# bigpon/QPNet

Measured on AMD Instinct MI355X. Metric: train steps/sec (batch-1 chunk-steps of RF+20000 samples, aggregate over GPUs), higher is better.
Workload: dtype f32; 1 GPU; config[1]: paper-size SI-QPNet (C=64,S=256,4F+4A) training step, forward+CE+backward+Adam on one chunk of 20900 samples (RF 946 + batch_length 19954), batch 1 per GPU; global_batch=1, parallelism=dp1 (utterance-sharded chunks, one flat-gradient all-reduce per step), backend=none, world_size=1, aux_1x1=frame rate (hoisted: K = 128 + one 4-deep step)

## Files before the change

qpnet_amd/csrc/train_bwd.hip:

```cpp
#include "train_common.h"
#include "train_post.h"
#include "qpn_handle.h"
#include <string.h>
#include <stdlib.h>
#include <math.h>

template <int MT>
__global__ __launch_bounds__(512) void k_post_bwd(TrainParams p, TrainBwd bw) {
    constexpr int TM = 16 * MT;
    extern __shared__ float sm[];
    const int S = p.S, Q = p.Q, LC = p.LC;
    const int ldp = tr_lda(Q > S ? Q : S), ldr = tr_lda(S);
    float* P = sm; float* R = sm + TM * ldp;
    const int b = blockIdx.y, t0 = blockIdx.x * TM;
    const int tid = threadIdx.x, lane = tid & 63, wave = tid >> 6;
    const int NTS = S / 16;
    const int npairs = (NTS + 1) / 2;
    const int np0 = wave < npairs ? wave : 0;
    const int pnt[2] = {2 * np0, (2 * np0 + 1 < NTS) ? 2 * np0 + 1 : 2 * np0};
    float my[2][MT][4], ms[2][MT][4];
    auto mask_load = [&](const float* src, float (&m)[2][MT][4]) {
#pragma unroll
        for (int j = 0; j < 2; ++j)
#pragma unroll
// ... 964 lines not shown
            a += ((v[0] + v[1]) + (v[2] + v[3])) + ((v[4] + v[5]) + (v[6] + v[7]));
        }
        for (; c < nch; ++c) a += sp[(size_t)c * gstage];
        a *= scale;
        for (int k = k0; k < k1; ++k) g[gdst_list[k]] = a;
        return;
    }
    if (!tail) return;
    const int64_t j = i - s1;
    if (j < n_gzero) g[gzero[j]] = 0.f;
    else if (append_scale && j < n_gzero + 4 && !(flag_again && j == n_gzero + 1)) g[n + (j - n_gzero)] = j == n_gzero ? scale : (j == n_gzero + 1 && status && *status) ? 1.f : 0.f;
}

__global__ __launch_bounds__(256) void k_causal_bwd(TrainParams p, TrainBwd bw, int rows_per_wg, int CB) {
    extern __shared__ float tab[];
    const int C = p.C, Q = p.Q;
    const int tid = threadIdx.x;
    const int64_t total = (int64_t)p.B * p.N1;
    const int64_t r0 = (int64_t)blockIdx.x * rows_per_wg, r1 = r0 + rows_per_wg < total ? r0 + rows_per_wg : total;
    for (int cb = 0; cb < C; cb += CB) {
        const int cbv = C - cb < CB ? C - cb : CB;
        for (int i = tid; i < 2 * Q * CB; i += 256) tab[i] = 0.f;
        __syncthreads();
        const int cpr = cbv;
        for (int64_t idx = r0 * cpr + tid; idx < r1 * cpr; idx += 256) {
            const int64_t rr = idx / cpr; const int c = (int)(idx - rr * cpr);
            const int b = (int)(rr / p.N1), n = (int)(rr - (int64_t)b * p.N1);
            const size_t o = ((size_t)b * p.N1 + n) * C + cb + c;
            const float v = bw.DXA[0][o] + bw.DXB[0][o];
            const int64_t xo = (int64_t)p.T - p.N0 + n;
            int64_t s0 = p.x[(size_t)b * p.T + xo] % Q, s1 = p.x[(size_t)b * p.T + xo + 1] % Q;
            if (s0 < 0) s0 += Q;
            if (s1 < 0) s1 += Q;
            atomicAdd(&tab[(0 * Q + s0) * CB + c], v);
            atomicAdd(&tab[(1 * Q + s1) * CB + c], v);
        }
        __syncthreads();
        for (int i = tid; i < 2 * Q * cbv; i += 256) {
            const int c = i / (2 * Q), qt = i - c * 2 * Q, q = qt >> 1, tp = qt & 1;
            const float v = tab[(tp * Q + q) * CB + c];
            if (v != 0.f) atomicAdd(&bw.gflat[p.causal_w + ((size_t)(cb + c) * Q + q) * 2 + tp], v * bw.gscale);
        }
        for (int c = tid; c < cbv; c += 256) {
            float s = 0.f;
            for (int q = 0; q < Q; ++q) s += tab[(0 * Q + q) * CB + c];
            atomicAdd(&bw.gflat[p.causal_b + cb + c], s * bw.gscale);
        }
        __syncthreads();
    }
}

__global__ __launch_bounds__(128) void k_up_bwd(UpArgs u) { up_bwd_body(u, blockIdx.x, blockIdx.y, threadIdx.x, 128); }

__global__ __launch_bounds__(128) void k_aux_tail(AuxArgs p) {
    __shared__ float hrow[1024];
    __shared__ float red[2];
    const AuxGeom& ag = p.g;
    const int C = p.C, A = p.A, L = p.L, tid = threadIdx.x;
    const int bx = blockIdx.x;
    float v = 0.f;
    const bool role_a = bx < L * A;
    if (role_a) {
        const int l = bx / A, a = bx - l * A, n = tid;
        const size_t wi = (n < C ? ag.auxS[l] + (size_t)n * A : ag.auxT[l] + (size_t)(n - C) * A) + a;
        const float va = p.flat[wi];
        float e = 0.f;
        {
            float ev[TR_EB_SLOTS];
#pragma unroll
            for (int k = 0; k < TR_EB_SLOTS; ++k) ev[k] = p.EB[(size_t)(l * TR_EB_SLOTS + k) * 2 * C + n];
#pragma unroll
            for (int k = 0; k < TR_EB_SLOTS; ++k) e += ev[k];
        }
        float acc = 0.f;
        for (int b = 0; b < p.B; ++b) {
            const float* hb = p.h + ((size_t)b * A + a) * p.F + p.ffirst;
            const float* D = p.DPA + (size_t)(l * p.B + b) * (p.nfr + 1) * 2 * C + n;
            for (int f0 = 0; f0 < p.nfr; f0 += 1024) {
                const int nf = p.nfr - f0 < 1024 ? p.nfr - f0 : 1024;
                __syncthreads();
                for (int i = tid; i < nf; i += 128) hrow[i] = hb[f0 + i];
                __syncthreads();
                int f = 0;
                for (; f + 64 <= nf; f += 64) {
                    float d[64];
#pragma unroll
                    for (int k = 0; k < 64; ++k) d[k] = D[(size_t)(f0 + f + k) * 2 * C];
#pragma unroll
                    for (int k = 0; k < 64; ++k) acc += d[k] * hrow[f + k];
                }
                for (; f + 16 <= nf; f += 16) {
                    float d[16];
#pragma unroll
                    for (int k = 0; k < 16; ++k) d[k] = D[(size_t)(f0 + f + k) * 2 * C];
#pragma unroll
                    for (int k = 0; k < 16; ++k) acc += d[k] * hrow[f + k];
                }
                for (; f < nf; ++f) acc += D[(size_t)(f0 + f) * 2 * C] * hrow[f];
            }
        }
        p.gflat[wi] = (acc + p.flat[p.up_b] * e) * p.gscale;
        v = va * e;
    } else {
        const int j = bx - L * A;
        const int q0 = p.F * p.U - p.N1;
        const int items = L * p.B * p.nfr;
        for (int it = tid; it < items; it += 128) {
            const int fx = it % p.nfr, lb = it / p.nfr, l = lb / p.B;
            const int n = (p.ffirst + fx) * p.U + j - q0;
            if (n >= ag.s_out[l] && n < p.N1) v += p.GW[(size_t)lb * p.N1 + n];
        }
    }
    for (int sft = 32; sft >= 1; sft >>= 1) v += __shfl_xor(v, sft);
    if ((tid & 63) == 0) red[tid >> 6] = v;
    __syncthreads();
    if (tid == 0) {
        if (role_a) atomicAdd(p.gflat + p.up_b, (red[0] + red[1]) * p.gscale);
        else p.gflat[p.up_w + (bx - L * A)] = (red[0] + red[1]) * p.gscale;
    }
}

__device__ __forceinline__ void zero_dx_slice(const TrainParams& p, const TrainBwd& bw, int j, int b, size_t part, size_t nparts, int t, int nthr) {
    const int C = p.C;
    const TrLayer ly = p.layers[j];
    const size_t nDX = (size_t)p.B * p.N1 * C;
    float* A = bw.DXA[0] + (size_t)j * nDX + (size_t)b * p.N1 * C;
    float* Bq = bw.DXB[0] + (size_t)j * nDX + (size_t)b * p.N1 * C;
    const int a0 = j == 0 ? 0 : ly.s_in, a1 = ly.s_out;
    const int b0 = ly.adaptive ? 0 : p.N1 - ly.dilation, b1 = p.N1;
    const size_t na = (size_t)(a1 - a0) * C / 4, nb = (size_t)(b1 > b0 ? b1 - b0 : 0) * C / 4;
    const float4 z = make_float4(0.f, 0.f, 0.f, 0.f);
    const size_t nh = p.hoist ? (size_t)(p.nfr + 1) * 2 * C / 4 : (j == 0 ? (size_t)p.N1 * p.Ap / 4 : 0);
    const size_t ne = (p.hoist && b == 0) ? (size_t)TR_EB_SLOTS * 2 * C / 4 : 0;
    float* H = p.hoist ? bw.DPA + (size_t)(j * p.B + b) * (p.nfr + 1) * 2 * C : bw.DHUP + (size_t)b * p.N1 * p.Ap;
    for (size_t i = part * nthr + t; i < na + nb + nh + ne; i += nparts * nthr) {
        if (i < na) ((float4*)(A + (size_t)a0 * C))[i] = z;
        else if (i < na + nb) ((float4*)(Bq + (size_t)(b0 > 0 ? b0 : 0) * C))[i - na] = z;
        else if (i < na + nb + nh) ((float4*)H)[i - na - nb] = z;
        else ((float4*)(bw.EB + (size_t)j * TR_EB_SLOTS * 2 * C))[i - na - nb - nh] = z;
    }
}
__global__ void k_zero_dx(TrainParams p, TrainBwd bw) {
    zero_dx_slice(p, bw, blockIdx.y, blockIdx.z, blockIdx.x, gridDim.x, threadIdx.x, blockDim.x);
}

void qpn_launch_zero_dx(const TrainParams& p, const TrainBwd& bw, hipStream_t stream) {
    hipLaunchKernelGGL(k_zero_dx, dim3(64, p.L, p.B), dim3(256), 0, stream, p, bw);
}

static void launch_reduce_early(const TrainBwd& bw, hipStream_t st, int tail, int nch_side) {
    const TrainSlabs& sl = *bw.sl;
    const int64_t n = (int64_t)(sl.g_early1 - sl.g_early0) + (tail ? bw.n_gzero + 4 : 0);
    hipLaunchKernelGGL(k_reduce_grad_s, dim3((unsigned)((n + 255) / 256)), dim3(256), 0, st, bw.slab, bw.gdst, bw.gdst_list, bw.gzero, bw.n_gzero,
                       nch_side, bw.gstage, bw.n_params, bw.gflat, bw.gscale, bw.append_scale, sl.g_early0, sl.g_early1, 0, 0, tail, bw.status, 0);
}
static void launch_up_bwd(const TrainParams& p, const TrainBwd& bw, hipStream_t st) {
    const UpArgs u = up_args(p, bw);
    hipLaunchKernelGGL(k_up_bwd, dim3(u.nfr, p.B), dim3(128), 0, st, u);
}

static void launch_aux_tail(const TrainParams& p, const TrainBwd& bw, const AuxGeom& ag, hipStream_t st) {
    hipLaunchKernelGGL(k_aux_tail, dim3(p.L * p.A + p.U), dim3(128), 0, st, tr_aux_args(p, &bw, ag));
}

int qpn_launch_grad_tail(const TrainParams& p, const TrainBwd& bw, const AuxGeom* ag, hipStream_t stream, bool early_done, bool up_done) {
    const int C = p.C, Q = p.Q, B = p.B, N1 = p.N1;
    const TrainSlabs& sl = *bw.sl;
    hipLaunchKernelGGL(k_reduce_grad_s, dim3((unsigned)(((int64_t)bw.gstage + (up_done ? 0 : bw.n_gzero + 4) + 255) / 256)), dim3(256), 0, stream, bw.slab, bw.gdst, bw.gdst_list, bw.gzero, bw.n_gzero,
                       bw.nch, bw.gstage, bw.n_params, bw.gflat, bw.gscale, bw.append_scale, 0, bw.gstage, early_done ? sl.g_early0 : 0, early_done ? sl.g_early1 : 0, up_done ? 0 : 1, bw.status, bw.append_scale == 1 ? 1 : 0);
    {
        const int64_t total = (int64_t)B * N1;
        const int nwg = 128, rpw = (int)((total + nwg - 1) / nwg);
        if (sl.g_cw < 0) {
            int CB = C < 64 ? C : 64;
            while (CB > 1 && (size_t)2 * Q * CB * sizeof(float) > 128 * 1024) CB /= 2;
            const size_t lds_c = (size_t)2 * Q * CB * sizeof(float);
            if (lds_c > 160 * 1024) { qpn_set_error("causal-table gradient: n_quantize too large for the LDS histogram"); return QPN_EINVAL; }
            if (lds_c > 48 * 1024) QPN_HIP(hipFuncSetAttribute((const void*)k_causal_bwd, hipFuncAttributeMaxDynamicSharedMemorySize, (int)lds_c));
            hipLaunchKernelGGL(k_causal_bwd, dim3(nwg), dim3(256), lds_c, stream, p, bw, rpw, CB);
        }
        if (p.U > 0 && !up_done && !p.hoist) launch_up_bwd(p, bw, stream);
        if (p.hoist && ag && !up_done) launch_aux_tail(p, bw, *ag, stream);
        if (bw.dh && !up_done) qpn_launch_input_grad(p, bw, ag, stream);
    }
    qpn_prof_mark(PG_GRAD_TAIL, stream);
    QPN_HIP(hipGetLastError());
    return QPN_OK;
}

bool qpn_stack_bwd_fits(const TrainParams& p);
int qpn_launch_stack_bwd(const TrainParams& p, const TrainBwd& bw, const StackQ& q, const TrainKnobs& k, hipStream_t stream);

void qpn_launch_post_fb(const TrainParams& p, const TrainBwd& bw, hipStream_t stream) {
    constexpr int MTW = 5;
    const size_t ldsw = (size_t)16 * MTW * (tr_lda(256) + 2 * tr_lda(64)) * sizeof(float);
    (void)hipFuncSetAttribute((const void*)k_post_fb_w<MTW>, hipFuncAttributeMaxDynamicSharedMemorySize, (int)ldsw);
    hipLaunchKernelGGL((k_post_fb_w<MTW>), dim3((p.BL + 16 * MTW - 1) / (16 * MTW), p.B), dim3(512), ldsw, stream, p, bw, 1);
}

int qpn_launch_bwd(const TrainParams& p, const TrainBwd& bw, const TrainKnobs& k, const AuxGeom& ag, const StackQ* sq, hipStream_t stream, bool post_done) {
    const int C = p.C, S = p.S, Q = p.Q, L = p.L, B = p.B, N1 = p.N1, BL = p.BL;
    const TrainSlabs& sl = *bw.sl;
    const bool off32 = N1 < (1 << 24) && (int64_t)N1 * (p.LC > 2 * C ? p.LC : 2 * C) < (1ll << 32);
    const bool persist = C == 64 && (p.Ktp == 176 || p.hoist) && p.Ap <= 64 && off32 && k.persist_bwd;
    const bool stack_q = persist && k.stack_q_bwd && sq && sq->flags && p.qctl && qpn_stack_bwd_fits(p);
    const bool wr_summed = stack_q;
    const size_t nDX = (size_t)B * N1 * C;
    const size_t lds_post = (size_t)16 * (tr_lda(Q > S ? Q : S) + tr_lda(S)) * sizeof(float);
    const size_t lds_layer = (size_t)16 * (4 * tr_lda(C) + tr_lda(2 * C)) * sizeof(float);
    if (lds_post > 160 * 1024 || lds_layer > 160 * 1024) { qpn_set_error("backward tiles do not fit LDS"); return QPN_EINVAL; }
    hipStream_t side = bw.side; hipEvent_t ev_fork = bw.ev_fork, ev_join = bw.ev_join;
    const bool overlap = side && !qpn_prof_serial() && !k.serial;
    const bool post_wide = S == 256 && Q == 256 && C == 64 && (p.LC == 256 || p.LC == 512) && k.post_wide;
    const bool zero_in_post = post_wide && k.zero_in_post;
    if (post_done) { }
    else if (!zero_in_post) qpn_launch_zero_dx(p, bw, stream);
    if (post_done) { }
    else if (post_wide) {
        constexpr int MTW = 5;
        const size_t ldsw = (size_t)16 * MTW * tr_lda(256) * sizeof(float);
        QPN_HIP(hipFuncSetAttribute((const void*)k_post_bwd_w<MTW>, hipFuncAttributeMaxDynamicSharedMemorySize, (int)ldsw));
        hipLaunchKernelGGL((k_post_bwd_w<MTW>), dim3((BL + 16 * MTW - 1) / (16 * MTW), B), dim3(512), ldsw, stream, p, bw, zero_in_post ? 1 : 0);
    } else {
        if (lds_post > 48 * 1024) (void)hipFuncSetAttribute((const void*)k_post_bwd<1>, hipFuncAttributeMaxDynamicSharedMemorySize, (int)lds_post);
        hipLaunchKernelGGL((k_post_bwd<1>), dim3((BL + 15) / 16, B), dim3(512), lds_post, stream, p, bw);
    }
    qpn_prof_mark(PG_POST_BWD, stream);
    const int nch = bw.nch;
    int nch_side_ = nch;
    const bool gen = k.wgrad_generic;
    Wg2 wbase; memset(&wbase, 0, sizeof(wbase));
    wbase.slab = bw.slab; wbase.gstage = bw.gstage; wbase.nb = B; wbase.C = C; wbase.Ap = p.Ap; wbase.hup = p.HUP; wbase.tap = p.TAP; wbase.ncol_groups = 1;
    bool ok = true;
    auto launch_skip_post = [&](hipStream_t st) {
        Wg2 w = wbase;
// ... 55 lines not shown
    }
    if (overlap) {
        QPN_HIP(hipEventRecord(ev_fork, stream));
        QPN_HIP(hipStreamWaitEvent(side, ev_fork, 0));
        qpn_prof_mark(-1, side);
        launch_skip_post(side);
        if (early_reduce) { launch_reduce_early(bw, side, up_side ? 1 : 0, nch_side_); qpn_prof_mark(PG_GRAD_TAIL, side); }
        if (early_reduce && up_side && bw.ev_early && bw.early_recorded) { QPN_HIP(hipEventRecord(bw.ev_early, side)); *bw.early_recorded = 1; }
    }
    const int swz = k.xcd_swizzle ? 1 : 0;
    if (p.hoist && !persist) { qpn_set_error("internal: the frame-rate aux term needs the register-resident layer kernels"); return QPN_EINVAL; }
    if (stack_q) {
        const int rcq = qpn_launch_stack_bwd(p, bw, *sq, k, stream);
        if (rcq) return rcq;
    }
    for (int l = L - 1; l >= 0 && !stack_q; --l) {
        const TrLayer& ly = p.layers[l];
        const int rows = N1 - ly.s_out;
        const int tiles = (rows + 15) / 16;
        if (persist) {
            int G = qpn_num_cus() * 2; if (G > tiles) G = tiles;
            if (G > 1024) G = 1024;
            const size_t ldsp = (size_t)(8 * 16 * tr_lda(C) + 16 * tr_lda(2 * C) + 16 * tr_lda(p.Ktp) + 64) * sizeof(float);
            const bool last = l == L - 1;
            const void* kf = p.hoist ? (last ? (const void*)k_layer_bwd_p<8, true> : (const void*)k_layer_bwd_p<8, false>)
                                     : (last ? (const void*)k_layer_bwd_p<11, true> : (const void*)k_layer_bwd_p<11, false>);
            (void)hipFuncSetAttribute(kf, hipFuncAttributeMaxDynamicSharedMemorySize, (int)ldsp);
            if (p.hoist) {
                if (last) hipLaunchKernelGGL((k_layer_bwd_p<8, true>), dim3(G, B), dim3(256), ldsp, stream, p, bw, l, swz ? 2 : 0, tiles, p.scratch_rows);
                else hipLaunchKernelGGL((k_layer_bwd_p<8, false>), dim3(G, B), dim3(256), ldsp, stream, p, bw, l, swz ? 2 : 0, tiles, p.scratch_rows);
            } else {
                if (last) hipLaunchKernelGGL((k_layer_bwd_p<11, true>), dim3(G, B), dim3(256), ldsp, stream, p, bw, l, swz ? 2 : 0, tiles, p.scratch_rows);
                else hipLaunchKernelGGL((k_layer_bwd_p<11, false>), dim3(G, B), dim3(256), ldsp, stream, p, bw, l, swz ? 2 : 0, tiles, p.scratch_rows);
            }
        } else {
            if (lds_layer > 48 * 1024) (void)hipFuncSetAttribute((const void*)k_layer_bwd<1>, hipFuncAttributeMaxDynamicSharedMemorySize, (int)lds_layer);
            hipLaunchKernelGGL((k_layer_bwd<1>), dim3(tiles, B), dim3(256), lds_layer, stream, p, bw, l, l == L - 1 ? 1 : 0, swz);
        }
    }
    auto build_causal = [&]() {
        Wg2 w = wbase;
        w.nlayers = 2; w.ncol_groups = Q / (Q % 64 == 0 ? 64 : 128);      w.bmode = 4; w.xc = p.XC; w.B1 = w.B2 = nullptr; w.B_lstride = 0;
        w.A = bw.DXA[0]; w.A2 = bw.DXB[0]; w.A_lstride = 0; w.lda = C; w.M = C; w.rowsA = N1;
        w.N = Q; w.Nvalid = Q; w.rowsB = N1 + 1; w.ldb = 0; w.ldc = Q;
        for (int tp = 0; tp < 2; ++tp) { w.row0A[tp] = 0; w.row0B[tp] = tp; w.R[tp] = N1; w.goff[tp] = sl.g_cw + tp * C * Q; w.gbias[tp] = tp == 0 ? sl.g_cb : -1; w.tap_off[tp] = -1; w.dil[tp] = 0; }
        return w;
    };
    const bool wr_side = overlap && k.wr_side;
    if (wr_side || up_side) {
        QPN_HIP(hipEventRecord(bw.ev_mid, stream));
        QPN_HIP(hipStreamWaitEvent(side, bw.ev_mid, 0));
        qpn_prof_mark(-1, side);
        if (up_side) {
            if (p.hoist) launch_aux_tail(p, bw, ag, side); else launch_up_bwd(p, bw, side);
            if (bw.dh) qpn_launch_input_grad(p, bw, &ag, side);
            qpn_prof_mark(PG_GRAD_TAIL, side);
        }
        if (wr_side) { ok = ok && wgrad2_any(build_wr(), nch, gen, side); qpn_prof_mark(PG_WGRAD_WR, side); }
    }
    if (overlap) QPN_HIP(hipEventRecord(ev_join, side));
    qpn_prof_mark(PG_LAYER_BWD, stream);
    ok = ok && wgrad2_any(build_w1(), nch, gen, stream);
    qpn_prof_mark(PG_WGRAD, stream);
    if (!wr_side) { ok = ok && wgrad2_any(build_wr(), nch, gen, stream); qpn_prof_mark(PG_WGRAD_WR, stream); }
    if (!overlap) launch_skip_post(stream);
    if (sl.g_cw >= 0) ok = ok && wgrad2_any(build_causal(), nch, gen, stream);
    qpn_prof_mark(PG_WGRAD_CAUSAL, stream);
    if (overlap) { QPN_HIP(hipStreamWaitEvent(stream, ev_join, 0)); qpn_prof_mark(-1, stream); }
    if (!ok) { qpn_set_error("weight-gradient tiles: unsupported geometry (n_resch <= 128 on this path; wider stacks take the GEMM path)"); return QPN_EINVAL; }
    return qpn_launch_grad_tail(p, bw, &ag, stream, early_reduce, up_side);
}
```

qpnet_amd/csrc/train_gemm.hip:

```cpp
#include "train_common.h"
#include "qpn_handle.h"
#include <string.h>

typedef float f32x16 __attribute__((ext_vector_type(16)));

#define GM 128
#define GN 128
#ifndef GK
#define GK 16
#endif
#ifndef GKT
#define GKT 16
#endif
#define G_LDA (GK + 1)
#ifndef GEMM_WAVES
#define GEMM_WAVES
#endif
#define G_LDB 128

enum { AL_PLAIN = 0, AL_SUM2 = 1, AL_RELU = 2 };
enum { EP_BIAS = 0, EP_GATE, EP_RES, EP_MASK, EP_DZ, EP_DA, EP_STORE };

struct GArgs {
    int M, N, K, nb;
// ... 401 lines not shown
    { AuxGeom ag0; memset(&ag0, 0, sizeof(ag0)); qpn_launch_prep(p, ag0, stream); }
    qpn_prof_mark(PG_PREP, stream);
    for (int l = 0; l < L; ++l) {
        const TrLayer& ly = p.layers[l];
        const int rows = N1 - ly.s_out;
        {
            GArgs g = gbase(p);
            g.M = rows; g.N = 2 * C; g.K = w.K1; g.row_base = ly.s_out;
            const float* Xin = p.X + (size_t)l * nDX;
            g.a[0] = Xin; g.a_ld[0] = C; g.a_kend[0] = C; g.a_kvalid[0] = C; g.a_tap[0] = 0; g.a_row0[0] = ly.s_out; g.a_bs[0] = (long)N1 * C;
            g.a[1] = Xin; g.a_ld[1] = C; g.a_kend[1] = 2 * C; g.a_kvalid[1] = C; g.a_tap[1] = 1; g.a_row0[1] = 0; g.a_bs[1] = (long)N1 * C;
            g.a[2] = p.HUP; g.a_ld[2] = p.Ap; g.a_kend[2] = w.K1; g.a_kvalid[2] = p.Ap; g.a_tap[2] = 0; g.a_row0[2] = ly.s_out; g.a_bs[2] = (long)N1 * p.Ap;
            g.tap = ly.adaptive ? p.TAP + ly.tap_off : nullptr; g.tap_bs = N1; g.dil = ly.dilation;
            g.b = w.wp + w.w1[l]; g.ldb = w.N1g;
            g.bias = p.bp + ly.bias1;
            g.o[0] = p.SG + (size_t)l * nDX; g.o[1] = p.TH + (size_t)l * nDX; g.o[2] = w.G + (size_t)l * nDX; g.o_bs = (long)N1 * C; g.o_ld = C; g.o_row0 = ly.s_out;
            launch_nn<AL_PLAIN, EP_GATE>(g, w.N1g / GN, stream);
        }
        if (l + 1 < L) {
            GArgs g = gbase(p);
            g.M = rows; g.N = C; g.K = C; g.row_base = ly.s_out;
            g.a[0] = w.G + (size_t)l * nDX; g.a_ld[0] = C; g.a_kvalid[0] = C; g.a_row0[0] = ly.s_out; g.a_bs[0] = (long)N1 * C;
            g.b = w.wp + w.wr[l]; g.ldb = w.Cg;
            g.bias = p.bp + ly.biasr;
            g.o[0] = p.X + (size_t)(l + 1) * nDX; g.o_bs = (long)N1 * C; g.o_ld = C; g.o_row0 = ly.s_out;
            g.e[0] = p.X + (size_t)l * nDX; g.e_bs = (long)N1 * C; g.e_ld = C; g.e_row0 = ly.s_out;
            launch_nn<AL_PLAIN, EP_RES>(g, w.Cg / GN, stream);
        }
    }
    qpn_prof_mark(PG_LAYER_FWD, stream);
    {
        GArgs g = gbase(p);
        g.M = BL; g.N = S; g.K = L * C; g.row_base = N1 - BL;
        g.a[0] = w.G; g.a_ld[0] = C; g.a_kvalid[0] = L * C; g.a_row0[0] = N1 - BL; g.a_bs[0] = (long)N1 * C;
        g.a_rep_len = C; g.a_rep_stride = (long)nDX;
        g.b = w.wp + w.ws; g.ldb = w.Sg; g.bias = p.bp + p.bias_s;
        g.o[0] = p.S0; g.o_bs = (long)BL * S; g.o_ld = S; g.o_row0 = 0;
        launch_nn<AL_PLAIN, EP_BIAS>(g, w.Sg / GN, stream);
        g = gbase(p);
        g.M = BL; g.N = S; g.K = S; g.a[0] = p.S0; g.a_ld[0] = S; g.a_kvalid[0] = S; g.a_bs[0] = (long)BL * S;
        g.b = w.wp + w.p1; g.ldb = w.Sg; g.bias = p.bp + p.bias_p1;
        g.o[0] = p.Y0; g.o_bs = (long)BL * S; g.o_ld = S;
        launch_nn<AL_RELU, EP_BIAS>(g, w.Sg / GN, stream);
        g.N = Q; g.a[0] = p.Y0; g.b = w.wp + w.p2; g.ldb = w.Qg; g.bias = p.bp + p.bias_p2;
        g.o[0] = p.logits; g.o_bs = (long)BL * Q; g.o_ld = Q;
        launch_nn<AL_RELU, EP_BIAS>(g, w.Qg / GN, stream);
    }
    qpn_prof_mark(PG_POST_FWD, stream);
    QPN_HIP(hipGetLastError());
    return QPN_OK;
}

void qpn_launch_zero_dx(const TrainParams& p, const TrainBwd& bw, hipStream_t stream);
int qpn_launch_grad_tail(const TrainParams& p, const TrainBwd& bw, const AuxGeom* ag, hipStream_t stream, bool early_done, bool up_done);

static void launch_post_wgrad_gemm(const TrainParams& p, const TrainBwd& bw, hipStream_t stream) {
    TArgs a; memset(&a, 0, sizeof(a));
    a.nb = p.B; a.nsplit = bw.nch; a.slab = bw.slab; a.gstage = bw.gstage; a.C = p.C; a.Ap = p.Ap;
    a.M = p.Q; a.N = p.S; a.a = bw.dlogits; a.lda = p.Q; a.rowsA = p.BL; a.b1 = p.Y0; a.ldb = p.S; a.rowsB = p.BL; a.ldc = p.S;
    a.R[0] = p.BL; a.goff[0] = bw.sl->g_p2; a.gbias[0] = bw.sl->g_bp2; a.tap_off[0] = -1;
    launch_tn<BM_RELU>(a, 1, stream);
    a.M = p.S; a.a = bw.DY0; a.lda = p.S; a.b1 = p.S0; a.goff[0] = bw.sl->g_p1; a.gbias[0] = bw.sl->g_bp1;
    launch_tn<BM_RELU>(a, 1, stream);
}

int qpn_launch_bwd_gemm(const TrainParams& p, const TrainBwd& bw, const TrainGemm& w, hipStream_t stream) {
    const int C = p.C, S = p.S, Q = p.Q, L = p.L, B = p.B, N1 = p.N1, BL = p.BL;
    const size_t nDX = (size_t)B * N1 * C;
    qpn_launch_zero_dx(p, bw, stream);
    {
        GArgs g = gbase(p);
        g.M = BL; g.N = S; g.K = Q; g.a[0] = bw.dlogits; g.a_ld[0] = Q; g.a_kvalid[0] = Q; g.a_bs[0] = (long)BL * Q;
        g.b = w.wp + w.p2t; g.ldb = w.Sg;
        g.o[0] = bw.DY0; g.o_bs = (long)BL * S; g.o_ld = S; g.e[0] = p.Y0; g.e_bs = (long)BL * S; g.e_ld = S;
        launch_nn<AL_PLAIN, EP_MASK>(g, w.Sg / GN, stream);
        g.K = S; g.a[0] = bw.DY0; g.a_ld[0] = S; g.a_kvalid[0] = S; g.a_bs[0] = (long)BL * S;
        g.b = w.wp + w.p1t; g.o[0] = bw.DS0; g.e[0] = p.S0;
        launch_nn<AL_PLAIN, EP_MASK>(g, w.Sg / GN, stream);
        g = gbase(p);
        g.M = BL; g.N = L * C; g.K = S; g.a[0] = bw.DS0; g.a_ld[0] = S; g.a_kvalid[0] = S; g.a_bs[0] = (long)BL * S;
        g.b = w.wp + w.wst; g.ldb = w.LCg;
        g.o[0] = bw.DGS; g.o_bs = (long)BL * L * C; g.o_ld = L * C;
        launch_nn<AL_PLAIN, EP_STORE>(g, w.LCg / GN, stream);
    }
    qpn_prof_mark(PG_POST_BWD, stream);
    for (int l = L - 1; l >= 0; --l) {
        const TrLayer& ly = p.layers[l];
        const int rows = N1 - ly.s_out;
        const bool last = l == L - 1;
        float* DZl = bw.DZ + (size_t)l * B * N1 * 2 * C;
        {
            GArgs g = gbase(p);
            g.M = rows; g.N = C; g.K = last ? 0 : C; g.row_base = ly.s_out;
            g.a[0] = bw.DXA[0] + (size_t)(l + 1) * nDX; g.a2 = bw.DXB[0] + (size_t)(l + 1) * nDX;
            g.a_ld[0] = C; g.a_kvalid[0] = C; g.a_row0[0] = ly.s_out; g.a_bs[0] = (long)N1 * C;
            g.b = w.wp + w.wrt[l]; g.ldb = w.Cg;
            g.o[0] = DZl; g.o_bs = (long)N1 * 2 * C; g.o_ld = 2 * C; g.o_row0 = ly.s_out;
            g.e[0] = p.SG + (size_t)l * nDX; g.e[1] = p.TH + (size_t)l * nDX; g.e_bs = (long)N1 * C; g.e_ld = C; g.e_row0 = ly.s_out;
            g.e3 = bw.DGS; g.e3_bs = (long)BL * L * C; g.e3_ld = L * C; g.e3_col0 = l * C; g.e3_rowmin = N1 - BL;
            launch_nn<AL_SUM2, EP_DZ>(g, w.Cg / GN, stream);
        }
        {
            GArgs g = gbase(p);
            g.M = rows; g.N = 2 * C + p.Ap; g.K = 2 * C; g.row_base = ly.s_out;
            g.a[0] = DZl; g.a_ld[0] = 2 * C; g.a_kvalid[0] = 2 * C; g.a_row0[0] = ly.s_out; g.a_bs[0] = (long)N1 * 2 * C;
            g.b = w.wp + w.w1t[l]; g.ldb = w.Ktg;
            g.tap = ly.adaptive ? p.TAP + ly.tap_off : nullptr; g.tap_bs = N1; g.dil = ly.dilation; g.adaptive = ly.adaptive; g.last = last;
            g.o[0] = bw.DXA[0] + (size_t)l * nDX; g.o_bs = (long)N1 * C; g.o_ld = C;
            g.e[0] = bw.DXA[0] + (size_t)(l + 1) * nDX; g.e[1] = bw.DXB[0] + (size_t)(l + 1) * nDX; g.e_bs = (long)N1 * C; g.e_ld = C; g.e_row0 = ly.s_out;
            g.db = bw.DXB[0] + (size_t)l * nDX; g.db_bs = (long)N1 * C;
            g.dh = bw.DHUP; g.dh_bs = (long)N1 * p.Ap;
            launch_nn<AL_PLAIN, EP_DA>(g, w.Ktg / GN, stream);
        }
    }
    qpn_prof_mark(PG_LAYER_BWD, stream);
    TArgs t; memset(&t, 0, sizeof(t));
    t.nb = B; t.nsplit = bw.nch; t.slab = bw.slab; t.gstage = bw.gstage; t.hup = p.HUP; t.tap = p.TAP; t.C = C; t.Ap = p.Ap;
    {
        TArgs a = t;
        a.M = 2 * C; a.N = 2 * C + p.Ap; a.a = bw.DZ; a.a_ls = (long)B * N1 * 2 * C; a.lda = 2 * C; a.rowsA = N1;
        a.b1 = p.X; a.b_ls = (long)nDX; a.ldb = C; a.rowsB = N1; a.ldc = p.Ktp;
        for (int l = 0; l < L; ++l) {
            const TrLayer& ly = p.layers[l];
            a.row0A[l] = a.row0B[l] = ly.s_out; a.R[l] = N1 - ly.s_out; a.goff[l] = bw.sl->g_w1[l]; a.gbias[l] = bw.sl->g_b1[l];
            a.tap_off[l] = ly.adaptive ? ly.tap_off : -1; a.dil[l] = ly.dilation;
        }
        launch_tn<BM_GATHER>(a, L, stream);
    }
    {
        TArgs a = t;
        a.M = C; a.N = C; a.a = bw.DXA[0] + nDX; a.a2 = bw.DXB[0] + nDX; a.a_ls = (long)nDX; a.lda = C; a.rowsA = N1;
        a.b1 = w.G; a.b_ls = (long)nDX; a.ldb = C; a.rowsB = N1; a.ldc = C;
        for (int l = 0; l < L; ++l) {
            a.row0A[l] = a.row0B[l] = p.layers[l].s_out; a.R[l] = l == L - 1 ? 0 : N1 - p.layers[l].s_out;
            a.goff[l] = bw.sl->g_wr[l]; a.gbias[l] = bw.sl->g_br[l]; a.tap_off[l] = -1;
        }
        launch_tn<BM_PLAIN>(a, L, stream);
    }
    {
        TArgs a = t;
        a.M = S; a.N = C; a.a = bw.DS0; a.a_ls = 0; a.lda = S; a.rowsA = BL;
        a.b1 = w.G; a.b_ls = (long)nDX; a.ldb = C; a.rowsB = N1; a.ldc = C;
        for (int l = 0; l < L; ++l) { a.row0A[l] = 0; a.row0B[l] = N1 - BL; a.R[l] = BL; a.goff[l] = bw.sl->g_ws[l]; a.gbias[l] = l == 0 ? bw.sl->g_bs : -1; a.tap_off[l] = -1; }
        launch_tn<BM_PLAIN>(a, L, stream);
    }
    launch_post_wgrad_gemm(p, bw, stream);
    qpn_prof_mark(PG_WGRAD, stream);
    return qpn_launch_grad_tail(p, bw, nullptr, stream, false, false);
}
```

qpnet_amd/csrc/train_host.hip:

```cpp
#include "train_common.h"
#include "qpn_handle.h"
#include <algorithm>
#include <memory>
#include <string.h>

int qpn_launch_fwd(const TrainParams& p, const TrainKnobs& k, const AuxGeom& ag, const StackQ* sq, hipStream_t stream, const TrainBwd* fuse_post_bwd, const RefreshArgs* rf);
bool qpn_step_prep_fits(const TrainParams& p);
void qpn_stack_fill(TrainParams& p);
static CeOpts ce_opts_of(const qpn_loss_opts& o, double* mass, double* d_mass);
int qpn_launch_bwd(const TrainParams& p, const TrainBwd& bw, const TrainKnobs& k, const AuxGeom& ag, const StackQ* sq, hipStream_t stream, bool post_done);
int qpn_launch_fwd_gemm(const TrainParams& p, const TrainGemm& w, hipStream_t stream);
int qpn_launch_bwd_gemm(const TrainParams& p, const TrainBwd& bw, const TrainGemm& w, hipStream_t stream);

#define LOSS_SLOT 72
static double loss_sum(const double* parts) { double sum = 0.0; for (int i = 0; i < 64; ++i) sum += parts[i]; return sum; }

struct TrainState {
    TrainLayout lay;
    int64_t n_map = 0;
    int* d_wmap = nullptr; float* d_wp = nullptr; int* d_bstart = nullptr; int* d_blist = nullptr; float* d_bp = nullptr;
    int* d_gdst = nullptr; int* d_gdst_list = nullptr; int* d_gzero = nullptr; int n_gzero = 0;
    TrainParams tp = {};
    TrainBwd bw = {};
    TrainKnobs knobs = {};
// ... 3 lines not shown
    double* d_loss3 = nullptr;
    double* d_mass = nullptr;
    int* d_status = nullptr; double* d_loss = nullptr;
    hipStream_t last_stream = nullptr;
    int* h_status_pinned = nullptr; hipEvent_t ev_status[2] = {}; bool status_pending[2] = {}; int status_newest = 0;
    double* h_loss_pinned = nullptr; hipEvent_t ev_loss[2] = {}; bool loss_pending[2] = {}; int loss_newest = 0;
    double* d_gnorm = nullptr; bool gnorm_last = false;
    bool gnorm_slot[2] = {};
    double gnorm_collected = 0.0; bool gnorm_collected_valid = false;
    bool fwd_valid = false;
    bool loss_clear = false;
    int* d_ctmap = nullptr; float* d_ct = nullptr;
    int* d_gmap = nullptr; float* d_gwp = nullptr;
    TrainGemm gm = {};
    int64_t generation = 0;
    hipStream_t side = nullptr; hipEvent_t ev_fork = nullptr, ev_join = nullptr, ev_mid = nullptr;
    hipEvent_t ev_early = nullptr; int early_recorded = 0;
    int64_t bwd_generation = -1;
    const float* post_bwd_dlogits = nullptr;
    bool post_bwd_done = false;
    bool stack_disabled = false;
    unsigned* d_sq = nullptr; size_t sq_pos_cap = 0, sq_per_dir = 0;
    StackQ sqf = {}, sqb = {};
};

static int env_int(const char* name, int dflt) { const char* e = getenv(name); return (e && *e) ? atoi(e) : dflt; }
void qpn_train_knobs_parse(TrainKnobs& k) {
    k.serial = env_int("QPN_TRAIN_SERIAL", 0) != 0;
    k.stack_q_fwd = env_int("QPN_STACK_QUEUE", 1) != 0;
    k.stack_q_bwd = k.stack_q_fwd && env_int("QPN_STACK_QUEUE_BWD", 1) != 0;
    k.stack_wgs = env_int("QPN_STACK_WGS", 0); if (k.stack_wgs < 0 || k.stack_wgs > 4096) k.stack_wgs = 0;
    k.stack_wgs_bwd = env_int("QPN_STACK_WGS_BWD", 0); if (k.stack_wgs_bwd < 0 || k.stack_wgs_bwd > 4096) k.stack_wgs_bwd = 0;
    k.persist_fwd = env_int("QPN_LAYER_PERSIST", 1) != 0;
    k.persist_bwd = env_int("QPN_LAYER_BWD_PERSIST", 1) != 0;
    k.wgrad_generic = getenv("QPN_WGRAD_GENERIC") != nullptr;
    k.wgrad_chunks = env_int("QPN_WGRAD_CHUNKS", 0); if (k.wgrad_chunks < 1 || k.wgrad_chunks > 512) k.wgrad_chunks = 0;
    k.wgrad_chunks_side = env_int("QPN_WGRAD_CHUNKS_SIDE", 0); if (k.wgrad_chunks_side < 1 || k.wgrad_chunks_side > 512) k.wgrad_chunks_side = 0;
    k.up_side = env_int("QPN_UP_SIDE", 1) != 0;
    k.reduce_early = env_int("QPN_REDUCE_EARLY", 1) != 0;
    k.wr_side = env_int("QPN_WR_SIDE", 1) != 0;
    k.post_fuse = env_int("QPN_POST_FUSE", 1) != 0;
    k.post_pair = env_int("QPN_POST_WGRAD_PAIR", 1) != 0;
    k.zero_in_post = env_int("QPN_ZERO_IN_POST", 1) != 0;
    k.post_wide = env_int("QPN_POST_WIDE", 1) != 0;
    k.xcd_swizzle = getenv("QPN_NO_XCD_SWIZZLE") == nullptr;
    k.ce_separate = getenv("QPN_CE_SEPARATE") != nullptr;
    k.event_fence = env_int("QPN_EVENT_FENCE", 0) == 1;
    k.aux_hoist = env_int("QPN_AUX_HOIST", 1) != 0;
    k.prep_fuse = env_int("QPN_PREP_FUSE", 1) != 0;
    k.test_stack_gives_up = false;
#ifdef QPN_TESTING
    k.test_stack_gives_up = env_int("QPN_TEST_STACK_GIVES_UP", 0) == 1;
#endif
}

int qpn_num_cus() {
    static int cached[64] = {0};
    int dev = 0;
    if (hipGetDevice(&dev) != hipSuccess || dev < 0 || dev >= 64) return 256;
    if (!cached[dev]) { int n = 0; if (hipDeviceGetAttribute(&n, hipDeviceAttributeMultiprocessorCount, dev) != hipSuccess || n < 1) n = 256; cached[dev] = n; }
    return cached[dev];
}

struct Prof { bool on = false; bool overlapped = false; std::vector<hipEvent_t> ev; std::vector<int> grp; std::vector<hipStream_t> st; size_t used = 0; };
static thread_local Prof g_prof;
bool qpn_prof_active() { return g_prof.on; }
bool qpn_prof_serial() { return g_prof.on && !g_prof.overlapped; }
void qpn_prof_mark(int group, hipStream_t stream) {
    Prof& P = g_prof;
    if (!P.on) return;
    if (P.used == P.ev.size()) { hipEvent_t e; if (hipEventCreate(&e) != hipSuccess) return; P.ev.push_back(e); P.grp.push_back(0); P.st.push_back(nullptr); }
    P.grp[P.used] = group; P.st[P.used] = stream;
    (void)hipEventRecord(P.ev[P.used++], stream);
}
extern "C" int qpn_train_profile_begin(qpn_handle* h, void* stream) {
    (void)h; g_prof.on = true; g_prof.overlapped = false; g_prof.used = 0;
    qpn_prof_mark(-1, (hipStream_t)stream);
    return QPN_OK;
}
extern "C" int qpn_train_profile_begin_overlapped(qpn_handle* h, void* stream) {
    (void)h; g_prof.on = true; g_prof.overlapped = true; g_prof.used = 0;
    qpn_prof_mark(-1, (hipStream_t)stream);
    return QPN_OK;
}
extern "C" int qpn_train_profile_mark(qpn_handle* h, int group, void* stream) {
    (void)h; qpn_prof_mark(group, (hipStream_t)stream); return QPN_OK;
}
extern "C" int qpn_train_profile_end(qpn_handle* h, float* h_ms, int n, void* stream) {
    Prof& P = g_prof;
    QPN_HIP(hipStreamSynchronize((hipStream_t)stream));
    if (h && h->train && h->train->side) QPN_HIP(hipStreamSynchronize(h->train->side));
    for (int i = 0; i < n; ++i) h_ms[i] = 0.f;
    for (size_t i = 1; i < P.used; ++i) {
        if (P.grp[i] < 0 || P.grp[i] >= n) continue;
        size_t j = i;
        while (j > 0 && P.st[j - 1] != P.st[i]) --j;
        if (j == 0) continue;
        float ms = 0.f;
        QPN_HIP(hipEventElapsedTime(&ms, P.ev[j - 1], P.ev[i]));
        h_ms[P.grp[i]] += ms;
    }
    P.on = false;
    return QPN_OK;
}

__global__ void k_gather_f(const float* __restrict__ flat, const int* __restrict__ map, float* __restrict__ out, int64_t n) {
// ... 823 lines not shown
```

qpnet_amd/csrc/train_plan.h:

```cpp
#pragma once
#include "qpn_geom.h"
#include <vector>

#define TR_MAXL QPN_MAX_LAYERS
#define TR_EB_SLOTS 32

struct TrainSlabs {
    int g_w1[TR_MAXL], g_b1[TR_MAXL], g_wr[TR_MAXL], g_br[TR_MAXL], g_ws[TR_MAXL], g_bs;
    int g_p1, g_bp1, g_p2, g_bp2;
    int g_early0, g_early1;
    int g_cw, g_cb;
};

struct AuxGeom { int auxS[TR_MAXL], auxT[TR_MAXL], bias1[TR_MAXL], s_out[TR_MAXL]; };

struct TrainGemm {
    const float* wp;
    float* G;
    int K1;
    int N1g, Cg, Sg, Qg, LCg, Ktg;
    long w1[TR_MAXL], w1t[TR_MAXL], wr[TR_MAXL], wrt[TR_MAXL];
    long ws, wst, p1, p1t, p2, p2t;
};

struct TrainKnobs {
    bool serial;
    bool stack_q_fwd, stack_q_bwd;
    int stack_wgs, stack_wgs_bwd;
    bool persist_fwd, persist_bwd;
    bool wgrad_generic;
    int wgrad_chunks, wgrad_chunks_side;
    bool post_fuse;
    bool up_side, reduce_early, wr_side;
    bool post_pair, zero_in_post, post_wide;
    bool xcd_swizzle;
    bool ce_separate;
    bool event_fence;
    bool prep_fuse;
    bool aux_hoist;
    bool test_stack_gives_up;
};

inline int64_t tp_causal_src(const Geom& g, int c, int q, int tap) { return g.causal_w + ((int64_t)c * g.Q + q) * 2 + tap; }
inline int tp_pad_to(int v, int q) { return (v + q - 1) / q * q; }

inline size_t tp_frag_pos(int N, int k, int n) {
    const int ks4 = k / 16, e = (k % 16) / 4, lane = ((k % 4) << 4) | (n % 16);
    return (((size_t)ks4 * (N / 16) + n / 16) * 64 + lane) * 4 + e;
}
template <class F>
inline int tp_frag_pack(std::vector<int>& map, int K, int N, bool transposed, F src) {
    const int off4 = (int)(map.size() / 4);
    map.resize(map.size() + (size_t)K * N);
    int* m = map.data() + (size_t)off4 * 4;
    for (int k = 0; k < K; ++k)
        for (int n = 0; n < N; ++n) m[tp_frag_pos(N, k, n)] = tp_idx(transposed ? src(n, k) : src(k, n));
    return off4;
}
template <class F>
inline long tp_kmajor_pack(std::vector<int>& map, int K, int Kp, int N, int Np, bool transposed, F src) {
    const long off = (long)map.size();
    map.resize(map.size() + (size_t)Kp * Np, -1);
    int* m = map.data() + off;
    for (int k = 0; k < K; ++k)
        for (int n = 0; n < N; ++n) m[(size_t)k * Np + n] = tp_idx(transposed ? src(n, k) : src(k, n));
    return off;
}
inline int tp_gemm_gate_col(int C, int q) {
    const int tile = q / 128, w = q % 128, half = w / 64, c = 64 * tile + w % 64;
    return c < C ? half * C + c : -1;
}

struct TrainPlanLayer { int adaptive, dilation, w1_f4, wr_f4, w1t_f4, wrt_f4, bias1, biasr; };
struct TrainLayout {
    bool use_gemm = false, hoist = false;
    int Ap = 0, Kt = 0, Ktp = 0, LC = 0;
    TrainPlanLayer layers[TR_MAXL] = {};
    int ws_f4 = 0, p1_f4 = 0, p2_f4 = 0, wst_f4 = 0, p1t_f4 = 0, p2t_f4 = 0, bias_s = 0, bias_p1 = 0, bias_p2 = 0;
    int n_bias = 0;
    TrainSlabs slabs = {};
    int gstage = 0, nch = 0;
    int64_t early_first = -1;
};
struct TrainPlan : TrainLayout {
    int rc = QPN_OK;
    AuxGeom ag = {};
    TrainGemm gm = {};
    std::vector<int> h_wmap;
    std::vector<int> h_gmap;
    std::vector<int> h_bstart, h_blist;
    std::vector<int> h_gsrc;
    std::vector<int> gdst_start, gdst_list;
    std::vector<int> gzero;
// ... 160 lines not shown
```

Baseline: 1497 steps/s.

## Tile aux-tail weight gradient over frames and batch several aux outputs per block

Replaces the one-block-per-(layer, aux output) aux tail kernel with a 256-thread kernel in which each block covers four aux outputs. It stages 64-frame tiles of the upstream gradient and the aux feature rows in LDS, prefetching the next tile into registers while the current one is consumed. This shares each loaded gradient tile across several outputs and cuts the block count and redundant global reads. The old kernel stays available behind QPN_TAIL_LEGACY. The new kernel is more complex and adds partial-tile edge handling.

Result: no change. 1499 steps/s, median of 2 (+0.1%).

```diff
diff --git a/qpnet_amd/csrc/train_bwd.hip b/qpnet_amd/csrc/train_bwd.hip
--- a/qpnet_amd/csrc/train_bwd.hip
+++ b/qpnet_amd/csrc/train_bwd.hip
@@ -1040,7 +1040,118 @@
 
 __global__ __launch_bounds__(128) void k_up_bwd(UpArgs u) { up_bwd_body(u, blockIdx.x, blockIdx.y, threadIdx.x, 128); }
 
-__global__ __launch_bounds__(128) void k_aux_tail(AuxArgs p) {
+template <int FBT>
+__global__ __launch_bounds__(256) void k_aux_tail(AuxArgs p) {
+    constexpr int FB = 2 * FBT, FT = 64, NH = (FB * FT + 255) / 256;
+    __shared__ __align__(16) float Dt[FT * 128];
+    __shared__ __align__(16) float hrow[FB * FT];
+    __shared__ float red[4 * FBT];
+    const AuxGeom& ag = p.g;
+    const int C = p.C, A = p.A, L = p.L, tid = threadIdx.x;
+    const int bx = blockIdx.x;
+    const int G = (A + FB - 1) / FB;
+    if (bx < L * G) {
+        const int l = bx / G, a0 = (bx - l * G) * FB;
+        const int n = tid & 127, q = tid >> 7;
+        size_t wi[FBT]; float va[FBT], acc[FBT];
+#pragma unroll
+        for (int j = 0; j < FBT; ++j) {
+            const int a = a0 + q * FBT + j;
+            wi[j] = (n < C ? ag.auxS[l] + (size_t)n * A : ag.auxT[l] + (size_t)(n - C) * A) + (a < A ? a : 0);
+            va[j] = p.flat[wi[j]]; acc[j] = 0.f;
+        }
+        float e = 0.f;
+        {
+            float ev[TR_EB_SLOTS];
+#pragma unroll
+            for (int k = 0; k < TR_EB_SLOTS; ++k) ev[k] = p.EB[(size_t)(l * TR_EB_SLOTS + k) * 2 * C + n];
+#pragma unroll
+            for (int k = 0; k < TR_EB_SLOTS; ++k) e += ev[k];
+        }
+        const int ntile = (p.nfr + FT - 1) / FT, nit = p.B * ntile;
+        const int drow = tid >> 5, dcol = (tid & 31) * 4;
+        f32x4 rd[8]; float rh[NH];
+        auto request = [&](int it) __attribute__((always_inline)) {
+            const int b = it / ntile, f0 = (it - b * ntile) * FT;
+            const float* Dl = p.DPA + (size_t)(l * p.B + b) * (p.nfr + 1) * 2 * C;
+#pragma unroll
+            for (int k = 0; k < 8; ++k) {
+                int r = f0 + drow + 8 * k; r = r < p.nfr ? r : p.nfr - 1;
+                rd[k] = *(const f32x4*)(Dl + (size_t)r * 2 * C + dcol);
+            }
+#pragma unroll
+            for (int k = 0; k < NH; ++k) {
+                const int idx = tid + 256 * k;
+                int j = idx / FT, f = f0 + (idx % FT);
+                int a = a0 + (j < FB ? j : FB - 1); a = a < A ? a : A - 1; f = f < p.nfr ? f : p.nfr - 1;
+                rh[k] = p.h[((size_t)b * A + a) * p.F + p.ffirst + f];
+            }
+        };
+        if (nit > 0) request(0);
+        for (int it = 0; it < nit; ++it) {
+            const int b = it / ntile, f0 = (it - b * ntile) * FT;
+            const int nf = p.nfr - f0 < FT ? p.nfr - f0 : FT;
+#pragma unroll
+            for (int k = 0; k < 8; ++k) *(f32x4*)(Dt + (drow + 8 * k) * 128 + dcol) = rd[k];
+#pragma unroll
+            for (int k = 0; k < NH; ++k) { const int idx = tid + 256 * k; if (idx < FB * FT) hrow[idx] = rh[k]; }
+            __syncthreads();
+            if (it + 1 < nit) request(it + 1);
+            const float* hq = hrow + q * FBT * FT;
+            if (nf == FT) {
+#pragma unroll 4
+                for (int k = 0; k < FT; k += 4) {
+                    float d[4]; float4 hv[FBT];
+#pragma unroll
+                    for (int i = 0; i < 4; ++i) d[i] = Dt[(k + i) * 128 + n];
+#pragma unroll
+                    for (int j = 0; j < FBT; ++j) hv[j] = *(const float4*)(hq + j * FT + k);
+#pragma unroll
+                    for (int j = 0; j < FBT; ++j) { acc[j] += d[0] * hv[j].x; acc[j] += d[1] * hv[j].y; acc[j] += d[2] * hv[j].z; acc[j] += d[3] * hv[j].w; }
+                }
+            } else {
+                for (int k = 0; k < nf; ++k) {
+                    const float d = Dt[k * 128 + n];
+#pragma unroll
+                    for (int j = 0; j < FBT; ++j) acc[j] += d * hq[j * FT + k];
+                }
+            }
+            __syncthreads();
+        }
+        const float bup = p.flat[p.up_b];
+#pragma unroll
+        for (int j = 0; j < FBT; ++j) {
+            const bool av = a0 + q * FBT + j < A;
+            if (av) p.gflat[wi[j]] = (acc[j] + bup * e) * p.gscale;
+            float v = av ? va[j] * e : 0.f;
+            for (int sft = 32; sft >= 1; sft >>= 1) v += __shfl_xor(v, sft);
+            if ((tid & 63) == 0) red[(tid >> 6) * FBT + j] = v;
+        }
+        __syncthreads();
+        if (tid < FB && a0 + tid < A) {
+            const int qq = tid / FBT, j = tid - qq * FBT;
+            atomicAdd(p.gflat + p.up_b, (red[(2 * qq) * FBT + j] + red[(2 * qq + 1) * FBT + j]) * p.gscale);
+        }
+    } else {
+        const int j = bx - L * G;
+        const int q0 = p.F * p.U - p.N1;
+        const int items = L * p.B * p.nfr;
+        float v = 0.f;
+        if (tid < 128)
+            for (int it = tid; it < items; it += 128) {
+                const int fx = it % p.nfr, lb = it / p.nfr, l = lb / p.B;
+                const int n = (p.ffirst + fx) * p.U + j - q0;
+                if (n >= ag.s_out[l] && n < p.N1) v += p.GW[(size_t)lb * p.N1 + n];
+            }
+        for (int sft = 32; sft >= 1; sft >>= 1) v += __shfl_xor(v, sft);
+        if ((tid & 63) == 0) red[tid >> 6] = v;
+        __syncthreads();
+        if (tid == 0) p.gflat[p.up_w + j] = (red[0] + red[1]) * p.gscale;
+    }
+}
+constexpr int AUX_TAIL_FBT = 2;
+
+__global__ __launch_bounds__(128) void k_aux_tail1(AuxArgs p) {
     __shared__ float hrow[1024];
     __shared__ float red[2];
     const AuxGeom& ag = p.g;
@@ -1147,11 +1258,13 @@
     hipLaunchKernelGGL(k_up_bwd, dim3(u.nfr, p.B), dim3(128), 0, st, u);
 }
 
-static void launch_aux_tail(const TrainParams& p, const TrainBwd& bw, const AuxGeom& ag, hipStream_t st) {
-    hipLaunchKernelGGL(k_aux_tail, dim3(p.L * p.A + p.U), dim3(128), 0, st, tr_aux_args(p, &bw, ag));
-}
-
-int qpn_launch_grad_tail(const TrainParams& p, const TrainBwd& bw, const AuxGeom* ag, hipStream_t stream, bool early_done, bool up_done) {
+static void launch_aux_tail(const TrainParams& p, const TrainBwd& bw, const AuxGeom& ag, bool legacy, hipStream_t st) {
+    constexpr int FB = 2 * AUX_TAIL_FBT;
+    if (legacy) hipLaunchKernelGGL(k_aux_tail1, dim3(p.L * p.A + p.U), dim3(128), 0, st, tr_aux_args(p, &bw, ag));
+    else hipLaunchKernelGGL(k_aux_tail<AUX_TAIL_FBT>, dim3(p.L * ((p.A + FB - 1) / FB) + p.U), dim3(256), 0, st, tr_aux_args(p, &bw, ag));
+}
+
+int qpn_launch_grad_tail(const TrainParams& p, const TrainBwd& bw, const AuxGeom* ag, hipStream_t stream, bool early_done, bool up_done, bool tail_legacy) {
     const int C = p.C, Q = p.Q, B = p.B, N1 = p.N1;
     const TrainSlabs& sl = *bw.sl;
     hipLaunchKernelGGL(k_reduce_grad_s, dim3((unsigned)(((int64_t)bw.gstage + (up_done ? 0 : bw.n_gzero + 4) + 255) / 256)), dim3(256), 0, stream, bw.slab, bw.gdst, bw.gdst_list, bw.gzero, bw.n_gzero,
@@ -1168,7 +1281,7 @@
             hipLaunchKernelGGL(k_causal_bwd, dim3(nwg), dim3(256), lds_c, stream, p, bw, rpw, CB);
         }
         if (p.U > 0 && !up_done && !p.hoist) launch_up_bwd(p, bw, stream);
-        if (p.hoist && ag && !up_done) launch_aux_tail(p, bw, *ag, stream);
+        if (p.hoist && ag && !up_done) launch_aux_tail(p, bw, *ag, tail_legacy, stream);
         if (bw.dh && !up_done) qpn_launch_input_grad(p, bw, ag, stream);
     }
     qpn_prof_mark(PG_GRAD_TAIL, stream);
@@ -1330,7 +1443,7 @@
         QPN_HIP(hipStreamWaitEvent(side, bw.ev_mid, 0));
         qpn_prof_mark(-1, side);
         if (up_side) {
-            if (p.hoist) launch_aux_tail(p, bw, ag, side); else launch_up_bwd(p, bw, side);
+            if (p.hoist) launch_aux_tail(p, bw, ag, k.tail_legacy, side); else launch_up_bwd(p, bw, side);
             if (bw.dh) qpn_launch_input_grad(p, bw, &ag, side);
             qpn_prof_mark(PG_GRAD_TAIL, side);
         }
@@ -1346,5 +1459,5 @@
     qpn_prof_mark(PG_WGRAD_CAUSAL, stream);
     if (overlap) { QPN_HIP(hipStreamWaitEvent(stream, ev_join, 0)); qpn_prof_mark(-1, stream); }
     if (!ok) { qpn_set_error("weight-gradient tiles: unsupported geometry (n_resch <= 128 on this path; wider stacks take the GEMM path)"); return QPN_EINVAL; }
-    return qpn_launch_grad_tail(p, bw, &ag, stream, early_reduce, up_side);
-}
+    return qpn_launch_grad_tail(p, bw, &ag, stream, early_reduce, up_side, k.tail_legacy);
+}
diff --git a/qpnet_amd/csrc/train_gemm.hip b/qpnet_amd/csrc/train_gemm.hip
--- a/qpnet_amd/csrc/train_gemm.hip
+++ b/qpnet_amd/csrc/train_gemm.hip
@@ -477,7 +477,7 @@
 }
 
 void qpn_launch_zero_dx(const TrainParams& p, const TrainBwd& bw, hipStream_t stream);
-int qpn_launch_grad_tail(const TrainParams& p, const TrainBwd& bw, const AuxGeom* ag, hipStream_t stream, bool early_done, bool up_done);
+int qpn_launch_grad_tail(const TrainParams& p, const TrainBwd& bw, const AuxGeom* ag, hipStream_t stream, bool early_done, bool up_done, bool tail_legacy);
 
 static void launch_post_wgrad_gemm(const TrainParams& p, const TrainBwd& bw, hipStream_t stream) {
     TArgs a; memset(&a, 0, sizeof(a));
@@ -571,5 +571,5 @@
     }
     launch_post_wgrad_gemm(p, bw, stream);
     qpn_prof_mark(PG_WGRAD, stream);
-    return qpn_launch_grad_tail(p, bw, nullptr, stream, false, false);
-}
+    return qpn_launch_grad_tail(p, bw, nullptr, stream, false, false, false);
+}
diff --git a/qpnet_amd/csrc/train_host.hip b/qpnet_amd/csrc/train_host.hip
--- a/qpnet_amd/csrc/train_host.hip
+++ b/qpnet_amd/csrc/train_host.hip
@@ -79,6 +79,7 @@
 #ifdef QPN_TESTING
     k.test_stack_gives_up = env_int("QPN_TEST_STACK_GIVES_UP", 0) == 1;
 #endif
+    k.tail_legacy = env_int("QPN_TAIL_LEGACY", 0) == 1;
 }
 
 int qpn_num_cus() {
diff --git a/qpnet_amd/csrc/train_plan.h b/qpnet_amd/csrc/train_plan.h
--- a/qpnet_amd/csrc/train_plan.h
+++ b/qpnet_amd/csrc/train_plan.h
@@ -39,6 +39,7 @@
     bool prep_fuse;
     bool aux_hoist;
     bool test_stack_gives_up;
+    bool tail_legacy;
 };
 
 inline int64_t tp_causal_src(const Geom& g, int c, int q, int tap) { return g.causal_w + ((int64_t)c * g.Q + q) * 2 + tap; }
```
